# marvinli00/genie2

Measured on AMD Instinct MI355X. Metric: denoise-steps/sec (N=256, T=1000, batch=8), higher is better.
Workload: dtype f32 (pair-stack products as 3 f16 MFMAs on 2xf16-split operands, f32 accumulate); 1 GPU; unconditional N=256, T=1000, batch=8 per GPU, random-init base Denoiser (15.7M params), scale=0.6, reverse-loop steps 995..676; parallelism=replica per GPU x1, no data-path collective

## Files before the change

### genie2_amd/csrc/genie_api.hip

```cpp
#include <stdio.h>
#include <stdlib.h>
#include <string.h>
#include <math.h>
#include <algorithm>
#include <cmath>
#include <new>
#include <string>
#include <vector>

#include "common.h"

void pair_kernels_init();
void pair_fused_kernels_init();
void single_kernels_init(const genie_dims_t& d, int n_max);
void launch_scale_copy(genie_ctx* h, hipStream_t st, const float* in, float* out, int n, float s);
size_t ipa_attn_lds(const genie_dims_t& d, int N);

static char g_create_err[512] = "";

void set_handle_free_error(const char* msg) { snprintf(g_create_err, sizeof g_create_err, "%s", msg); }

#define SET_ERR(h, ...) do { snprintf((h)->err, sizeof((h)->err), __VA_ARGS__); } while (0)
#define HIP_TRY(h, call) do { hipError_t e_ = (call); if (e_ != hipSuccess) { \
    SET_ERR(h, "%s failed: %s (%s:%d)", #call, hipGetErrorString(e_), __FILE__, __LINE__); return GENIE_E_HIP; } } while (0)
// ... 100 lines not shown
static void free_batch(genie_ctx* h) {
    if (h->ws) { (void)hipFree(h->ws); h->ws = nullptr; h->ws_bytes = 0; }
    h->have_feats = false;
}

void genie_destroy(genie_handle_t h) {
    if (!h) return;
    (void)hipSetDevice(h->device);
    free_batch(h);
    train_ws_free(h);
    if (h->wdev) (void)hipFree(h->wdev);
    if (h->hxdev) (void)hipFree(h->hxdev);
    if (h->pos_tab) (void)hipFree(h->pos_tab);
    free(h->sched_host);
    for (int i = 0; i < h->prof_n; ++i) { (void)hipEventDestroy(h->prof_recs[i].a); (void)hipEventDestroy(h->prof_recs[i].b); }
    free(h->prof_recs);
    if (h->st2) { (void)hipStreamSynchronize(h->st2); (void)hipEventDestroy(h->ev_fork); (void)hipEventDestroy(h->ev_join); (void)hipStreamDestroy(h->st2); }
    delete[] h->pair;
    delete[] h->st;
    delete h;
}

const char* genie_last_error(genie_handle_t h) { return h ? h->err : g_create_err; }
size_t genie_workspace_bytes(genie_handle_t h) { return h ? h->ws_bytes : 0; }

namespace {
struct Img {
    std::vector<float> data;
    size_t add(size_t n) {
        const size_t off = (data.size() + 63) & ~(size_t)63;
        data.resize(off + n, 0.f);
        return off;
    }
    size_t raw(const float* src, size_t n) { const size_t o = add(n); memcpy(&data[o], src, n * sizeof(float)); return o; }
    size_t pack(const float* W, int rows, int cols) {
        const int NB = (rows + 31) / 32, KB = (cols + 7) / 8;
        const size_t o = add((size_t)NB * KB * 256);
        float* p = &data[o];
        for (int nb = 0; nb < NB; ++nb)
            for (int kb = 0; kb < KB; ++kb)
                for (int lane = 0; lane < 64; ++lane)
                    for (int e = 0; e < 4; ++e) {
                        const int r = nb * 32 + (lane & 31), k = kb * 8 + 4 * (lane >> 5) + e;
                        p[(((size_t)nb * KB + kb) * 64 + lane) * 4 + e] = (r < rows && k < cols) ? W[(size_t)r * cols + k] : 0.f;
                    }
        return o;
    }
};
uint16_t f2h(float f) {
    uint32_t x; memcpy(&x, &f, 4);
    const uint16_t sign = (uint16_t)((x >> 16) & 0x8000);
    x &= 0x7FFFFFFFu;
    if (x >= 0x7F800000u) return (uint16_t)(sign | (x > 0x7F800000u ? 0x7E00 : 0x7C00));
    if (x >= 0x477FF000u) return (uint16_t)(sign | 0x7C00);
    if (x < 0x38800000u) {
        float a; memcpy(&a, &x, 4);
        return (uint16_t)(sign | (uint16_t)nearbyintf(a * 16777216.0f));
    }
    const uint32_t mant = x & 0x7FFFFFu, rem = mant & 0x1FFFu;
    uint32_t r = (((x >> 23) - 112u) << 10) | (mant >> 13);
    if (rem > 0x1000u || (rem == 0x1000u && (r & 1u))) ++r;
    return (uint16_t)(sign | r);
}
float h2f(uint16_t v) {
    const int e = (v >> 10) & 31, m = v & 1023;
    float r = e == 0 ? ldexpf((float)m, -24) : e == 31 ? (m ? NAN : INFINITY) : ldexpf((float)(1024 + m), e - 25);
    return (v & 0x8000) ? -r : r;
}
float p2floor(double x) { return (x > 0 && std::isfinite(x)) ? (float)ldexp(1.0, (int)floor(log2(x))) : 1.0f; }
struct HxImg {
    std::vector<uint16_t> d;
    size_t begin() { d.resize((d.size() + 127) & ~(size_t)127); return d.size() * 2; }
    template <class F> void unit(F get) {
        const size_t o = d.size();
        d.resize(o + 1024);
        for (int lane = 0; lane < 64; ++lane)
            for (int e = 0; e < 8; ++e) {
                const float v = get(lane & 31, lane >> 5, e);
                const uint16_t hi = f2h(v);
                d[o + lane * 8 + e] = hi;
                d[o + 512 + lane * 8 + e] = f2h(v - h2f(hi));
            }
    }
};
double max_abs(const float* w, size_t n) { double m = 0; for (size_t i = 0; i < n; ++i) m = std::max(m, (double)fabsf(w[i])); return m; }
double hx_bound(const float* W, const float* b, int rows, int cols) {
    double m = 0;
    for (int r = 0; r < rows; ++r) {
        double ss = 0;
        for (int k = 0; k < cols; ++k) ss += (double)W[(size_t)r * cols + k] * W[(size_t)r * cols + k];
        m = std::max(m, sqrt(ss * cols) + fabs((double)b[r]));
    }
    return m;
}
constexpr float HX_SX = 1024.0f;

struct Cur {
    const float* p; size_t left;
    const float* take(size_t n) { if (n > left) { left = 0; return nullptr; } const float* r = p; p += n; left -= n; return r; }
};
void fold_ln(std::vector<float>& W, std::vector<float>& b, int rows, int cols, const float* g, const float* beta) {
    for (int r = 0; r < rows; ++r) {
        double acc = b[r];
        for (int k = 0; k < cols; ++k) acc += (double)W[(size_t)r * cols + k] * beta[k];
        b[r] = (float)acc;
        for (int k = 0; k < cols; ++k) W[(size_t)r * cols + k] *= g[k];
    }
}
std::vector<float> vcat(std::initializer_list<std::pair<const float*, size_t>> parts) {
    std::vector<float> v;
    for (auto& pr : parts) v.insert(v.end(), pr.first, pr.first + pr.second);
    return v;
}
}

int genie_load_weights(genie_handle_t h, const float* blob, size_t n_floats) {
    if (!h || !blob) return GENIE_E_ARG;
    const genie_dims_t& d = h->d;
    if (n_floats != genie_weight_count(&d)) {
        SET_ERR(h, "genie_load_weights: got %zu floats, dims need %zu", n_floats, genie_weight_count(&d));
        return GENIE_E_ARG;
    }
    HIP_TRY(h, hipSetDevice(h->device));
    const size_t cs = d.c_s, cp = d.c_p, ch = d.c_hidden_mul;
    Cur c{blob, n_floats};
    Img img;
    HxImg hx;
    std::vector<std::pair<float**, size_t>> fix;
    std::vector<std::pair<const unsigned char**, size_t>> hxfix;
    auto slot = [&](float** s, size_t off) { fix.push_back({s, off}); };
    struct GemmFix { float** slot; size_t hx_off; float inv_s; };
    std::vector<GemmFix> gfix;
    auto pack_gemm = [&](float** s, const float* W, int rows, int cols) {
        slot(s, img.pack(W, rows, cols));
        const float sw = p2floor(16384.0 / max_abs(W, (size_t)rows * cols));
        gfix.push_back({s, hx.begin(), 1.0f / sw});
        const int NB = (rows + 31) / 32, KC = (cols + 15) / 16;
        for (int nb = 0; nb < NB; ++nb)
            for (int kc = 0; kc < KC; ++kc)
                hx.unit([&](int j, int hh, int e) {
                    const int r = 32 * nb + j, k = 16 * kc + 8 * hh + e;
                    return (r < rows && k < cols) ? W[(size_t)r * cols + k] * sw : 0.f; });
    };

    size_t ones_off, zeros_off;
    {
        std::vector<float> one(512, 1.f), zero(512, 0.f);
        ones_off = img.raw(one.data(), one.size());
        zeros_off = img.raw(zero.data(), zero.size());
    }
    const int nsi = single_in(d);
    pack_gemm(&h->single_w, c.take(cs * nsi), (int)cs, nsi);
    {
        const float* wi = c.take(cp * cs);
        const float* wj = c.take(cp * cs);
        auto v = vcat({{wi, cp * cs}, {wj, cp * cs}});
        pack_gemm(&h->pij_w, v.data(), (int)(2 * cp), (int)cs);
    }
    {
        const int nr = 2 * d.relpos_k + 3;
        const float* w = c.take(cp * nr);
        std::vector<float> t((size_t)nr * cp);
        for (int o = 0; o < (int)cp; ++o) for (int k = 0; k < nr; ++k) t[(size_t)k * cp + o] = w[(size_t)o * nr + k];
        slot(&h->relpos_t, img.raw(t.data(), t.size()));
    }
    {
// ... 62 lines not shown
                        for (int kc = 0; kc < 8; ++kc) {
                            const std::vector<float>& m = (st & 1) ? zw : gw;
                            const float sc = (st & 1) ? szo : sgo;
                            const size_t ob = 2 * (st >> 1) + obl;
                            hx.unit([&](int j, int hh, int e) { return m[(32 * ob + j) * cp + 16 * kc + 8 * hh + e] * sc; });
                        }
                std::vector<float> bp(4 * ch), bgs(cp), bzs(cp);
                for (size_t r = 0; r < 4 * ch; ++r) bp[r] = bb[r] * HX_SX * (r < 2 * ch ? sp : sg);
                for (size_t r = 0; r < cp; ++r) { bgs[r] = gb[r] * HX_SX * sgo; bzs[r] = zb[r] * HX_SX * szo; }
                slot(&X.bias_proj, img.raw(bp.data(), bp.size()));
                slot(&X.bgs, img.raw(bgs.data(), cp)); slot(&X.bzs, img.raw(bzs.data(), cp));
                tm_save[2 * l + dir] = TmSave{w, gw, zw, sp, sg, sgo, szo};
            }
            slot(&T.ln_in_g, ones_off); slot(&T.ln_in_b, zeros_off);
            slot(&T.ln_out_g, ones_off); slot(&T.ln_out_b, zeros_off);
        }
        for (int node = 0; node < (d.n_head_tri > 0 ? 2 : 0); ++node) {
            TriAttW& A = node == 0 ? L.ta_start : L.ta_end;
            const size_t hc = (size_t)d.n_head_tri * d.c_hidden_tri_att;
            const float* ln_g = c.take(cp); const float* ln_b = c.take(cp);
            const float* b_w = c.take(d.n_head_tri * cp);
            const float* q_w = c.take(hc * cp); const float* k_w = c.take(hc * cp); const float* v_w = c.take(hc * cp);
            const float* o_w = c.take(cp * hc); const float* o_b = c.take(cp);
            const float* g_w = c.take(hc * cp); const float* g_b = c.take(hc);
            if (!g_b) { SET_ERR(h, "genie_load_weights: blob too short"); return GENIE_E_ARG; }
            slot(&A.ln_g, img.raw(ln_g, cp)); slot(&A.ln_b, img.raw(ln_b, cp));
            slot(&A.wb, img.raw(b_w, d.n_head_tri * cp));
            auto w = vcat({{q_w, hc * cp}, {k_w, hc * cp}, {v_w, hc * cp}, {g_w, hc * cp}});
            std::vector<float> bv(4 * hc, 0.f);
            memcpy(&bv[3 * hc], g_b, hc * sizeof(float));
            pack_gemm(&A.proj_w, w.data(), (int)(4 * hc), (int)cp);
            slot(&A.proj_b, img.raw(bv.data(), bv.size()));
            pack_gemm(&A.out_w, o_w, (int)cp, (int)hc); slot(&A.out_b, img.raw(o_b, cp));
            auto scale_of = [&](const float* W) {
                std::vector<float> wf(W, W + hc * cp), bf(hc, 0.f);
                fold_ln(wf, bf, (int)hc, (int)cp, ln_g, ln_b);
                return p2floor(32768.0 / hx_bound(wf.data(), bf.data(), (int)hc, (int)cp));
            };
            A.sq = scale_of(q_w); A.sk = scale_of(k_w); A.sv = scale_of(v_w);
        }
        const size_t nh = (size_t)d.pair_transition_n * cp;
        const float* lg = c.take(cp); const float* lb = c.take(cp);
        const float* w1 = c.take(nh * cp); const float* b1 = c.take(nh);
        const float* w2 = c.take(cp * nh); const float* b2 = c.take(cp);
        {
            std::vector<float> w1v(w1, w1 + nh * cp), b1v(b1, b1 + nh);
            fold_ln(w1v, b1v, (int)nh, (int)cp, lg, lb);
            slot(&L.pt_ln_g, ones_off); slot(&L.pt_ln_b, zeros_off);
            slot(&L.pt_w1, img.pack(w1v.data(), (int)nh, (int)cp)); slot(&L.pt_b1, img.raw(b1v.data(), nh));
            HxTransW& X = L.hx_pt;
            const float s1 = p2floor(16384.0 / max_abs(w1v.data(), nh * cp)), s2 = p2floor(16384.0 / max_abs(w2, cp * nh));
            const float sh = p2floor(32768.0 / hx_bound(w1v.data(), b1v.data(), (int)nh, (int)cp));
            X.sx = HX_SX; X.c1 = sh / (HX_SX * s1); X.c2 = 1.0f / (sh * s2);
            hxfix.push_back({&X.img, hx.begin()});
            for (size_t hb = 0; hb < nh / 32; ++hb) {
                for (int kc = 0; kc < 8; ++kc)
                    hx.unit([&](int i, int hh, int e) { return w1v[(32 * hb + i) * cp + 16 * kc + 8 * hh + e] * s1; });
                for (int cc = 0; cc < 2; ++cc)
                    for (int ob = 0; ob < 4; ++ob)
                        hx.unit([&](int j, int hh, int e) {
                            return w2[(size_t)(32 * ob + j) * nh + 32 * hb + 16 * cc + (e & 3) + 8 * (e >> 2) + 4 * hh] * s2; });
            }
            std::vector<float> b1s(nh), b2s(cp);
            for (size_t r = 0; r < nh; ++r) b1s[r] = b1v[r] * HX_SX * s1;
            for (size_t r = 0; r < cp; ++r) b2s[r] = b2[r] * sh * s2;
            slot(&X.b1s, img.raw(b1s.data(), nh)); slot(&X.b2s, img.raw(b2s.data(), cp));
            pt_save[l] = PtSave{w1v, std::vector<float>(w2, w2 + cp * nh), s1, s2};
        }
        slot(&L.pt_w2, img.pack(w2, (int)cp, (int)nh)); slot(&L.pt_b2, img.raw(b2, cp));
    }
    {
        auto ck = [](int kc, int hh, int e) { return 16 * kc + (e & 3) + 8 * (e >> 2) + 4 * hh; };
        auto emit_O = [&](const TmSave& t) {
            for (int which = 0; which < 2; ++which)
                for (int st = 0; st < 2; ++st)
                    for (int obl = 0; obl < 2; ++obl)
                        for (int kc = 0; kc < 8; ++kc) {
                            const std::vector<float>& m = which == 0 ? t.zw : t.gw;
                            const float sc = which == 0 ? t.szo : t.sgo;
                            const size_t ob = 2 * st + obl;
                            hx.unit([&](int i, int hh, int e) { return m[(32 * ob + i) * cp + ck(kc, hh, e)] * sc; });
                        }
        };
        auto emit_T = [&](const PtSave& t) {
            const size_t nh = (size_t)d.pair_transition_n * cp;
            for (size_t hb = 0; hb < nh / 32; ++hb) {
                for (int kc = 0; kc < 8; ++kc)
                    hx.unit([&](int i, int hh, int e) { return t.w1v[(32 * hb + i) * cp + ck(kc, hh, e)] * t.s1; });
                for (int cc = 0; cc < 2; ++cc)
                    for (int ob = 0; ob < 4; ++ob)
                        hx.unit([&](int j, int hh, int e) { return t.w2[(size_t)(32 * ob + j) * nh + 32 * hb + ck(cc, hh, e)] * t.s2; });
            }
        };
        auto emit_P = [&](const TmSave& t) {
            for (size_t pass = 0; pass < 8; ++pass)
                for (int kc = 0; kc < 8; ++kc) {
                    hx.unit([&](int i, int hh, int e) { return t.w[(32 * pass + i) * cp + ck(kc, hh, e)] * t.sp; });
                    hx.unit([&](int i, int hh, int e) { return t.w[(2 * ch + 32 * pass + i) * cp + ck(kc, hh, e)] * t.sg; });
                }
        };
        for (int l = 0; l < d.n_pair_transform_layer; ++l) {
            hxfix.push_back({&h->pair[l].fa.img, hx.begin()});
            emit_O(tm_save[2 * l]); emit_P(tm_save[2 * l + 1]);
            hxfix.push_back({&h->pair[l].fb.img, hx.begin()});
            emit_O(tm_save[2 * l + 1]); emit_T(pt_save[l]);
            if (l + 1 < d.n_pair_transform_layer) emit_P(tm_save[2 * l + 2]);
        }
    }
    const size_t H = d.n_head_ipa, C = d.c_hidden_ipa, Pq = d.n_qk_point, Pv = d.n_v_point;
    const size_t ncat = ipa_cat_n(d);
    std::vector<float> wb_all, bb_all;
    for (int l = 0; l < d.n_structure_layer; ++l) {
        StructLayerW& S = h->st[l];
        const float* hw = c.take(H);
        const float* q_w = c.take(H * C * cs);            const float* q_b = c.take(H * C);
        const float* kv_w = c.take(2 * H * C * cs);       const float* kv_b = c.take(2 * H * C);
        const float* qp_w = c.take(3 * H * Pq * cs);      const float* qp_b = c.take(3 * H * Pq);
        const float* kp_w = c.take(3 * H * (Pq + Pv) * cs); const float* kp_b = c.take(3 * H * (Pq + Pv));
        const float* b_w = c.take(H * cp);                const float* b_b = c.take(H);
        const float* o_w = c.take(cs * ncat);             const float* o_b = c.take(cs);
        const float* li_g = c.take(cs); const float* li_b = c.take(cs);
        const float* t1w = c.take(cs * cs); const float* t1b = c.take(cs);
        const float* t2w = c.take(cs * cs); const float* t2b = c.take(cs);
        const float* t3w = c.take(cs * cs); const float* t3b = c.take(cs);
        const float* lt_g = c.take(cs); const float* lt_b = c.take(cs);
        const float* bw = c.take(6 * cs); const float* bbs = c.take(6);
        if (!bbs) { SET_ERR(h, "genie_load_weights: blob too short"); return GENIE_E_ARG; }
        slot(&S.head_w, img.raw(hw, H));
        auto w = vcat({{q_w, H * C * cs}, {kv_w, 2 * H * C * cs}, {qp_w, 3 * H * Pq * cs}, {kp_w, 3 * H * (Pq + Pv) * cs}});
        auto bv = vcat({{q_b, H * C}, {kv_b, 2 * H * C}, {qp_b, 3 * H * Pq}, {kp_b, 3 * H * (Pq + Pv)}});
        pack_gemm(&S.proj_w, w.data(), ipa_proj_n(d), (int)cs);
        slot(&S.proj_b, img.raw(bv.data(), bv.size()));
        wb_all.insert(wb_all.end(), b_w, b_w + H * cp);
        bb_all.insert(bb_all.end(), b_b, b_b + H);
        pack_gemm(&S.out_w, o_w, (int)cs, (int)ncat); slot(&S.out_b, img.raw(o_b, cs));
        slot(&S.ln_ipa_g, img.raw(li_g, cs)); slot(&S.ln_ipa_b, img.raw(li_b, cs));
        pack_gemm(&S.t1_w, t1w, (int)cs, (int)cs); slot(&S.t1_b, img.raw(t1b, cs));
        pack_gemm(&S.t2_w, t2w, (int)cs, (int)cs); slot(&S.t2_b, img.raw(t2b, cs));
        pack_gemm(&S.t3_w, t3w, (int)cs, (int)cs); slot(&S.t3_b, img.raw(t3b, cs));
        slot(&S.ln_tr_g, img.raw(lt_g, cs)); slot(&S.ln_tr_b, img.raw(lt_b, cs));
        slot(&S.bb_w, img.raw(bw, 6 * cs)); slot(&S.bb_b, img.raw(bbs, 6));
    }
    pack_gemm(&h->ipa_bias_w, wb_all.data(), (int)(d.n_structure_layer * H), (int)cp);
    slot(&h->ipa_bias_b, img.raw(bb_all.data(), bb_all.size()));
    if (c.left != 0) { SET_ERR(h, "genie_load_weights: %zu floats left over", c.left); return GENIE_E_ARG; }

    if (h->wdev) { (void)hipFree(h->wdev); h->wdev = nullptr; }
    img.add(64);
    HIP_TRY(h, hipMalloc((void**)&h->wdev, img.data.size() * sizeof(float)));
    HIP_TRY(h, hipMemcpy(h->wdev, img.data.data(), img.data.size() * sizeof(float), hipMemcpyHostToDevice));
    h->wdev_floats = img.data.size();
    for (auto& f : fix) *f.first = h->wdev + f.second;
    if (h->hxdev) { (void)hipFree(h->hxdev); h->hxdev = nullptr; }
    hx.begin();
    HIP_TRY(h, hipMalloc((void**)&h->hxdev, hx.d.size() * 2 + 256));
    HIP_TRY(h, hipMemcpy(h->hxdev, hx.d.data(), hx.d.size() * 2, hipMemcpyHostToDevice));
    for (auto& f : hxfix) *f.first = h->hxdev + f.second;
    h->n_hxg = 0;
    const int hxg_cap = (int)(sizeof(h->hxg) / sizeof(h->hxg[0]));
    if ((int)gfix.size() > hxg_cap) { SET_ERR(h, "genie_load_weights: %zu row-GEMM weights exceed the %d hx image slots", gfix.size(), hxg_cap); return GENIE_E_ARG; }
    for (auto& g : gfix) h->hxg[h->n_hxg++] = HxGemmW{*g.slot, h->hxdev + g.hx_off, g.inv_s};
    h->have_weights = true;
    return GENIE_OK;
}

int genie_set_tables(genie_handle_t h, const float* pos_tab, int n_pos, const float* chain_tab, int n_chain,
                     const float* t_tab, const float* sched) {
    if (!h || !pos_tab || !chain_tab || !t_tab || !sched || n_pos < 1 || n_chain < 1) return GENIE_E_ARG;
    HIP_TRY(h, hipSetDevice(h->device));
    const genie_dims_t& d = h->d;
    const size_t T1 = d.n_timestep + 1;
    const size_t a = (size_t)n_pos * d.c_pos_emb, b = (size_t)n_chain * d.c_chain_emb, c = T1 * d.c_timestep_emb, s = 4 * T1;
    if (h->pos_tab) (void)hipFree(h->pos_tab);
    HIP_TRY(h, hipMalloc((void**)&h->pos_tab, (a + b + c + s) * sizeof(float)));
// ... 374 lines not shown
```

### genie2_amd/csrc/hx.h

```cpp
#pragma once
#include "common.h"

#ifdef __HIPCC__
typedef _Float16 h8 __attribute__((ext_vector_type(8)));
typedef _Float16 h2 __attribute__((ext_vector_type(2)));
typedef unsigned u32x4 __attribute__((ext_vector_type(4)));

#define MFH(a, b, c) c = __builtin_amdgcn_mfma_f32_32x32x16_f16(a, b, c, 0, 0, 0)
#define MFH3(ah, al, bh, bl, c) do { MFH(al, bh, c); MFH(ah, bl, c); MFH(ah, bh, c); } while (0)

__device__ __forceinline__ void hx_split2(float a, float b, float s, unsigned& hi, unsigned& lo) {
    asm("v_fma_mixlo_f16 %0, %1, %2, 0" : "=v"(hi) : "v"(a), "v"(s));
    asm("v_fma_mixhi_f16 %0, %1, %2, 0" : "+v"(hi) : "v"(b), "v"(s));
    asm("v_fma_mixlo_f16 %0, %1, %2, -%3 op_sel_hi:[0,0,1]" : "=v"(lo) : "v"(a), "v"(s), "v"(hi));
    asm("v_fma_mixhi_f16 %0, %1, %2, -%3 op_sel:[0,0,1] op_sel_hi:[0,0,1]" : "+v"(lo) : "v"(b), "v"(s), "v"(hi));
}
__device__ __forceinline__ void hx_split8(const float (&x)[8], float s, h8& hi, h8& lo) {
    u32x4 h, l;
    unsigned a, b;
    hx_split2(x[0], x[1], s, a, b); h.x = a; l.x = b;
    hx_split2(x[2], x[3], s, a, b); h.y = a; l.y = b;
    hx_split2(x[4], x[5], s, a, b); h.z = a; l.z = b;
    hx_split2(x[6], x[7], s, a, b); h.w = a; l.w = b;
    hi = __builtin_bit_cast(h8, h);
    lo = __builtin_bit_cast(h8, l);
}
__device__ __forceinline__ unsigned hx_pack_prod(float u, float t) {
    unsigned w;
    asm("v_fma_mixlo_f16 %0, %1, %2, 0" : "=v"(w) : "v"(u), "v"(t));
    asm("v_fma_mixhi_f16 %0, %1, %2, -%0 op_sel_hi:[0,0,1]" : "+v"(w) : "v"(u), "v"(t));
    return w;
}
__device__ __forceinline__ h8 hx_frag(const unsigned char* stage, int u, int part, int lane) {
    return *reinterpret_cast<const h8*>(stage + u * 2048 + part * 1024 + lane * 16);
}
#endif

#define HX_STAGE_BYTES 32768
#define HX_UNITS 16
```

### genie2_amd/csrc/hx_fused.h

```cpp
#pragma once
#include "hx_pair.h"

#define FZ_SB_BZ 0
#define FZ_SB_BG 128
#define FZ_SB_B1 256
#define FZ_SB_B2 768
#define FZ_SB_BP 896
#define FZ_SB_FLOATS 1408
#define FZ_OOR 0x7FFFFFF0
#define FZ_COMPILER_FENCE() asm volatile("" ::: "memory")

struct FusedArgs {
    float* z; const float* xcm; const float* rmask; const unsigned char* wimg;
    const float *bzs, *bgs, *b1s, *b2s, *bproj;
    unsigned *acm, *bcm;
    int N, NP, n_wtiles, n_hb;
    unsigned cm_bytes, z_bytes;
    float sx, cgo, cz, c1, c2, inv_c2, cpa, cpb, cg;
    int rev;
};

__device__ __forceinline__ void fz_zt_read(float4 (&raw)[16], const unsigned char* zt, int pl, int h, int half) {
#pragma unroll
    for (int q = 0; q < 4; ++q) {
        const int g = 4 * q + h;
        raw[2 * (4 * half + q)] = *reinterpret_cast<const float4*>(zt + pl * 256 + ((g ^ (pl & 15)) << 4));
        raw[2 * (4 * half + q) + 1] = *reinterpret_cast<const float4*>(zt + pl * 256 + (((g + 2) ^ (pl & 15)) << 4));
    }
}

__device__ __forceinline__ void fz_zt_chunk(float4& a, float4& b, const unsigned char* zt, int pl, int h, int q) {
    const int g = 4 * q + h;
    a = *reinterpret_cast<const float4*>(zt + pl * 256 + ((g ^ (pl & 15)) << 4));
    b = *reinterpret_cast<const float4*>(zt + pl * 256 + (((g + 2) ^ (pl & 15)) << 4));
}

__device__ __forceinline__ void fz_store_half(rsrc_t rz, unsigned char* zt, const f32x16& v0, const f32x16& v1, int lane, int soff,
                                              int row_stride, int nvalid, int hf) {
    const int pl = lane & 31, h = lane >> 5;
    FZ_COMPILER_FENCE();
#pragma unroll
    for (int q = 0; q < 4; ++q) {
        const f32x16& v = (q < 2) ? v0 : v1;
        const int r0 = 8 * (q & 1);
        const int g = 4 * q + h;
        *reinterpret_cast<float4*>(zt + pl * 256 + ((g ^ (pl & 15)) << 4)) = make_float4(v[r0], v[r0 + 1], v[r0 + 2], v[r0 + 3]);
        *reinterpret_cast<float4*>(zt + pl * 256 + (((g + 2) ^ (pl & 15)) << 4)) = make_float4(v[r0 + 4], v[r0 + 5], v[r0 + 6], v[r0 + 7]);
    }
    hx_lds_done();
#pragma unroll
    for (int j = 0; j < 8; ++j) {
        const int r = 4 * j + (lane >> 4);
        u32x4 d = *reinterpret_cast<const u32x4*>(zt + j * 1024 + lane * 16);
        const int g = (lane & 15) ^ (r & 15);
        const int voff = r < nvalid ? r * row_stride + (g << 4) : FZ_OOR;
        __builtin_amdgcn_raw_buffer_store_b128(d, rz, voff, soff + hf * 256, 0);
        asm volatile("s_nop 1" : "+v"(d) : : "memory");
    }
    FZ_COMPILER_FENCE();
}

__device__ __forceinline__ void fz_stats(const f32x16 (&v)[4], float sx, float& mean, float& sc) {
    float s = 0.f;
#pragma unroll
    for (int ob = 0; ob < 4; ++ob)
#pragma unroll
        for (int r = 0; r < 16; ++r) s += v[ob][r];
    s += __shfl_xor(s, 32);
    mean = s * (1.0f / 128.0f);
    float ss = 0.f;
#pragma unroll
    for (int ob = 0; ob < 4; ++ob)
#pragma unroll
        for (int r = 0; r < 16; ++r) { const float d = v[ob][r] - mean; ss += d * d; }
    ss += __shfl_xor(ss, 32);
    sc = sx / sqrtf(ss * (1.0f / 128.0f) + GENIE_LN_EPS);
}
__device__ __forceinline__ void fz_split_tile(h8 (&zh)[8], h8 (&zl)[8], const f32x16 (&v)[4], float mean, float sc) {
#pragma unroll
    for (int c = 0; c < 8; ++c) {
        float x[8];
#pragma unroll
        for (int e = 0; e < 8; ++e) x[e] = v[c >> 1][8 * (c & 1) + e] - mean;
        hx_split8(x, sc, zh[c], zl[c]);
    }
}
```

### genie2_amd/csrc/pair_fused_kernels.hip

```cpp
#include <string.h>
#include "hx_fused.h"

#define FZ_LDS_BYTES (2 * HX_STAGE_BYTES + 6144 + 8 * HX_ZT_BYTES)

template <bool COL, bool HAS_T, bool HAS_P = true>
__global__ __launch_bounds__(512, 1) void k_pair_fused(const FusedArgs A) {
    extern __shared__ __attribute__((aligned(16))) unsigned char smb[];
    float* sb = reinterpret_cast<float*>(smb + 2 * HX_STAGE_BYTES);
    const int lane = threadIdx.x & 63, wave = UNI(threadIdx.x >> 6);
    const int h = lane >> 5, pl = lane & 31;
    const int N = A.N, NP = A.NP, n_wtiles = A.n_wtiles;
    const int ntile = (N + 31) >> 5;
    const int n_tiles = (n_wtiles + 7) / 8;
    const int rev = A.rev;
    const int n_hb = HAS_T ? A.n_hb : 0;
    const int PBASE = 4 + n_hb;
    const rsrc_t rw = hx_rsrc(A.wimg, (unsigned)((PBASE + (HAS_P ? 8 : 0)) * HX_STAGE_BYTES));
    const rsrc_t rx = hx_rsrc(A.xcm, A.cm_bytes), rz = hx_rsrc(A.z, A.z_bytes);
    const rsrc_t ra = hx_rsrc(A.acm, A.cm_bytes), rb = hx_rsrc(A.bcm, A.cm_bytes);
    const int lane16 = lane * 16;
    const int sstride = NP * NP * 4;
    const int zstride = COL ? N * 512 : 512;
    auto issue = [&](int s, int buf) {
        if (wave >= 4) {
// ... 96 lines not shown
#pragma unroll
                        for (int q = 0; q < 4; ++q) fz_zt_chunk(rz1[2 * q], rz1[2 * q + 1], zt, pl_t, h_t, q);
                    }
                    if (half == 0 && kc == 2) { hx_lds_done(); hx_zt_dma(rz, zt, lane_t, zsoff, zstride, znv, 0); }
                    if (half == 1 && kc == 1) {
                        zsh = __shfl(rz1[0].x, lane & 31);
#pragma unroll
                        for (int q = 0; q < 8; ++q) {
                            const float a = rz1[q].x - zsh, bq = rz1[q].y - zsh, c = rz1[q].z - zsh, d = rz1[q].w - zsh;
                            zs1 += (a + bq) + (c + d); zs2 += (a * a + bq * bq) + (c * c + d * d);
                        }
                    }
                    if (half == 1 && kc >= 2 && kc <= 5) {
                        float4 ta, tb;
                        fz_zt_chunk(ta, tb, zt, pl_t, h_t, kc - 2);
                        const float a = ta.x - zsh, bq = ta.y - zsh, c = ta.z - zsh, d = ta.w - zsh;
                        const float e = tb.x - zsh, f = tb.y - zsh, g = tb.z - zsh, hh = tb.w - zsh;
                        zs1 += ((a + bq) + (c + d)) + ((e + f) + (g + hh));
                        zs2 += ((a * a + bq * bq) + (c * c + d * d)) + ((e * e + f * f) + (g * g + hh * hh));
                    }
                }
                hx_stage_landed();
                hx_stage_barrier();
            }
            zs1 += __shfl_xor(zs1, 32); zs2 += __shfl_xor(zs2, 32);
            const float zm_s = zs1 * (1.0f / 128.0f);
            const float zmean = zsh + zm_s;
            const float zsc = A.sx / sqrtf(fmaxf(zs2 * (1.0f / 128.0f) - zm_s * zm_s, 0.f) + GENIE_LN_EPS);
#pragma unroll
            for (int half = 0; half < 2; ++half) {
                if (half == 0) issue(3, 1);
                else issue(4, 0);
                const unsigned char* stage = smb + half * HX_STAGE_BYTES;
                f32x16 ga, gb;
#pragma unroll
                for (int r = 0; r < 16; ++r) {
                    ga[r] = sbt[FZ_SB_BG + (2 * half) * 32 + acc_row(r, lane)];
                    gb[r] = sbt[FZ_SB_BG + (2 * half + 1) * 32 + acc_row(r, lane)];
                }
                h8 f0 = hx_frag(stage, 0, 0, lane), f0l = hx_frag(stage, 0, 1, lane), f1 = hx_frag(stage, 8, 0, lane),
                   f1l = hx_frag(stage, 8, 1, lane);
#pragma unroll
                for (int kc = 0; kc < 8; ++kc) {
                    const int kn = min(kc + 1, 7);
                    const h8 n0 = hx_frag(stage, kn, 0, lane), n0l = hx_frag(stage, kn, 1, lane), n1 = hx_frag(stage, 8 + kn, 0, lane),
                             n1l = hx_frag(stage, 8 + kn, 1, lane);
                    float4 ca, cb;
                    if (kc < 4) fz_zt_chunk(ca, cb, zt, pl_t, h_t, kc);
                    else { ca = rz1[2 * (kc - 4)]; cb = rz1[2 * (kc - 4) + 1]; }
                    const float xz[8] = {ca.x - zmean, ca.y - zmean, ca.z - zmean, ca.w - zmean, cb.x - zmean, cb.y - zmean, cb.z - zmean, cb.w - zmean};
                    h8 sh, sl;
                    hx_split8(xz, zsc, sh, sl);
                    PIPE_FENCE();
                    MFH3(f0, f0l, sh, sl, ga);
                    MFH3(f1, f1l, sh, sl, gb);
                    PIPE_FENCE();
                    f0 = n0; f0l = n0l; f1 = n1; f1l = n1l;
                }
                float4 res[8];
                if (half == 0) {
#pragma unroll
                    for (int q = 0; q < 4; ++q) fz_zt_chunk(res[2 * q], res[2 * q + 1], zt, pl_t, h_t, q);
                } else {
#pragma unroll
                    for (int q = 0; q < 8; ++q) res[q] = rz1[q];
                }
#pragma unroll
                for (int r = 0; r < 16; ++r) {
                    const float g0 = A.cz * __builtin_amdgcn_rcpf(1.0f + __builtin_amdgcn_exp2f(ga[r] * A.cgo));
                    const float g1 = A.cz * __builtin_amdgcn_rcpf(1.0f + __builtin_amdgcn_exp2f(gb[r] * A.cgo));
                    const float4 za = res[2 * (r >> 3) + ((r & 7) >> 2)], zb = res[2 * (2 + (r >> 3)) + ((r & 7) >> 2)];
                    const float z0 = (r & 3) == 0 ? za.x : (r & 3) == 1 ? za.y : (r & 3) == 2 ? za.z : za.w;
                    const float z1 = (r & 3) == 0 ? zb.x : (r & 3) == 1 ? zb.y : (r & 3) == 2 ? zb.z : zb.w;
                    v[2 * half][r] = fmaf(v[2 * half][r], g0, z0);
                    v[2 * half + 1][r] = fmaf(v[2 * half + 1][r], g1, z1);
                }
                hx_stage_landed();
                hx_stage_barrier();
            }
        }

        h8 zh[8], zl[8];
        if constexpr (HAS_T) {
            float mean, sc;
            fz_stats(v, A.sx, mean, sc);
            fz_split_tile(zh, zl, v, mean, sc);
#pragma unroll
            for (int ob = 0; ob < 4; ++ob)
#pragma unroll
                for (int r = 0; r < 16; ++r) v[ob][r] = fmaf(v[ob][r], A.inv_c2, sbt[FZ_SB_B2 + ob * 32 + acc_row(r, lane)]);
            f32x16 d;
#pragma unroll
            for (int r = 0; r < 16; ++r) d[r] = sbt[FZ_SB_B1 + acc_row(r, lane)];
            auto t_stage = [&](int hb) {
                if (HAS_P || hb + 1 < n_hb) issue(4 + hb + 1, (hb + 1) & 1);
                else if (more) issue(0, 0);
                const unsigned char* stage = smb + (hb & 1) * HX_STAGE_BYTES;
                {
                    h8 wh = hx_frag(stage, 0, 0, lane), wl = hx_frag(stage, 0, 1, lane);
#pragma unroll
                    for (int kc = 0; kc < 8; ++kc) {
                        const h8 nh = hx_frag(stage, min(kc + 1, 7), 0, lane), nl = hx_frag(stage, min(kc + 1, 7), 1, lane);
                        PIPE_FENCE();
                        MFH3(wh, wl, zh[kc], zl[kc], d);
                        PIPE_FENCE();
                        wh = nh; wl = nl;
                    }
                }
                h8 ah[2], al[2];
#pragma unroll
                for (int c = 0; c < 2; ++c) {
                    float x[8];
#pragma unroll
                    for (int e = 0; e < 8; ++e) x[e] = fmaxf(d[8 * c + e], 0.f);
                    hx_split8(x, A.c1, ah[c], al[c]);
                }
                {
                    h8 bh = hx_frag(stage, 8, 0, lane), bl = hx_frag(stage, 8, 1, lane);
#pragma unroll
                    for (int u = 0; u < 8; ++u) {
                        const h8 nh = hx_frag(stage, 8 + min(u + 1, 7), 0, lane), nl = hx_frag(stage, 8 + min(u + 1, 7), 1, lane);
                        PIPE_FENCE();
                        MFH3(bh, bl, ah[u >> 2], al[u >> 2], v[u & 3]);
                        PIPE_FENCE();
                        bh = nh; bl = nl;
                        if (u == 1) {
#pragma unroll
                            for (int r = 0; r < 16; ++r) d[r] = sbt[FZ_SB_B1 + (hb + 1) * 32 + acc_row(r, lane)];
                        }
                    }
                }
                hx_stage_landed();
                hx_stage_barrier();
            };
#pragma unroll 1
            for (int hb = 0; hb < n_hb; ++hb) t_stage(hb);
            const float m2 = msk * A.c2;
#pragma unroll
            for (int ob = 0; ob < 4; ++ob)
#pragma unroll
                for (int r = 0; r < 16; ++r) v[ob][r] *= m2;
        }

        fz_store_half(rz, zt, v[0], v[1], lane_t, zsoff, zstride, nvalid, 0);
        FZ_COMPILER_FENCE();
        fz_store_half(rz, zt, v[2], v[3], lane_t, zsoff, zstride, nvalid, 1);
        FZ_COMPILER_FENCE();
        if constexpr (HAS_P) {
            float mean, sc;
            fz_stats(v, A.sx, mean, sc);
            fz_split_tile(zh, zl, v, mean, sc);
        }
        hx_lds_done();
        if constexpr (!HAS_P) {
            if (more) hx_zt_dma(rz, zt, lane_t, n_zsoff, zstride, n_nv, 1);
        }

        if constexpr (HAS_P) {
            const float* sbias = sbt + FZ_SB_BP;
            const float cg = A.cg;
            const float ma = msk * A.cpa, mb = msk * A.cpb;
            const int voff = (pl < nvalid) ? (4 * h * NP * NP + pl) * 4 : FZ_OOR;
            const int sbase = ((b * 128 * NP + line) * NP + t0i) * 4;
            unsigned wst[8];
            f32x16 apA, agA, apB, agB;
#pragma unroll
            for (int r = 0; r < 16; ++r) { apB[r] = 0.f; agB[r] = 0.f; apA[r] = sbias[acc_row(r, lane)]; agA[r] = sbias[256 + acc_row(r, lane)]; }
#pragma unroll 1
            for (int pp = 0; pp < 4; ++pp) {
                {
                    const int pass = 2 * pp;
                    issue(PBASE + pass + 1, 1);
                    const unsigned char* stage = smb;
                    const rsrc_t e_rd = pp > 2 ? rb : ra;
                    const int e_voff = pp == 0 ? FZ_OOR : voff;
                    const int e_so = sbase + ((pass - 1) & 3) * 32 * sstride;
                    const float e_pm = pp > 2 ? mb : ma;
                    HX_PROJ_STAGE(apA, agA, apB, agB);
                    asm volatile("s_waitcnt vmcnt(16)" ::: "memory");
                    if (more) {
                        if (pp == 2) hx_zt_dma(rz, zt, lane_t, n_zsoff, zstride, n_nv, 1, 0, 4);
                    }
                    hx_stage_barrier();
                }
                {
                    const int pass = 2 * pp + 1;
                    if (pp < 3) issue(PBASE + pass + 1, 0);
                    else if (more) issue(0, 0);
                    const unsigned char* stage = smb + HX_STAGE_BYTES;
                    const rsrc_t e_rd = pp < 2 ? ra : rb;
                    const int e_voff = voff;
                    const int e_so = sbase + ((pass - 1) & 3) * 32 * sstride;
                    const float e_pm = pp < 2 ? ma : mb;
                    HX_PROJ_STAGE(apB, agB, apA, agA);
                    asm volatile("s_waitcnt vmcnt(16)" ::: "memory");
                    if (more) {
                        if (pp == 2) hx_zt_dma(rz, zt, lane_t, n_zsoff, zstride, n_nv, 1, 4, 4);
                    }
                    hx_stage_barrier();
                }
            }
            {
                const rsrc_t e_rd = rb;
                const int e_voff = voff, e_so = sbase + 3 * 32 * sstride;
                const float e_pm = mb;
                float t[16], u[16];
#pragma unroll
                for (int r = 0; r < 16; ++r) {
                    HX_PROJ_PIECE_A(agB, r, t[r]);
                    HX_PROJ_PIECE_B(apB, r, t[r], u[r]);
                }
                PIPE_FENCE();
#pragma unroll
                for (int r = 0; r < 16; ++r) HX_PROJ_PIECE_C_NOW(r, t[r], u[r]);
            }
        }
    }
#undef FZ_XLOAD
}

static int fz_num_cu() {
    static int n = 0;
    if (!n) { int dev = 0; hipDeviceProp_t pr; (void)hipGetDevice(&dev); (void)hipGetDeviceProperties(&pr, dev); n = pr.multiProcessorCount > 0 ? pr.multiProcessorCount : 256; }
    return n;
}

void pair_fused_kernels_init() {
    (void)hipFuncSetAttribute(reinterpret_cast<const void*>(k_pair_fused<true, false>), hipFuncAttributeMaxDynamicSharedMemorySize, FZ_LDS_BYTES);
    (void)hipFuncSetAttribute(reinterpret_cast<const void*>(k_pair_fused<false, true>), hipFuncAttributeMaxDynamicSharedMemorySize, FZ_LDS_BYTES);
    (void)hipFuncSetAttribute(reinterpret_cast<const void*>(k_pair_fused<false, true, false>), hipFuncAttributeMaxDynamicSharedMemorySize, FZ_LDS_BYTES);
// ... 23 lines not shown
```

Measured before the change: 110.7 batch-steps/s.

## Switch pair transition MLP to 16x16x32 MFMAs with transposed tile layout

Rewrites the pair-transition stage of the fused pair kernel to use 16x16x32 f16 MFMAs instead of 32x32x16. The accumulator tile is transposed through LDS into a new per-lane layout, and the host-side weight packing is re-emitted in matching 16-row units. The result is written back from that layout, with a round trip through LDS to restore the old register layout when the following projection needs it. This adds LDS shuffles, lane shuffles for the per-row stats, and recomputes the mask per element; the aim is presumably a better MFMA rate or better latency hiding for this shape.

Result: no change. 111.5 batch-steps/s (median of 6 runs) (+0.7%).

```diff
diff --git a/genie2_amd/csrc/genie_api.hip b/genie2_amd/csrc/genie_api.hip
--- a/genie2_amd/csrc/genie_api.hip
+++ b/genie2_amd/csrc/genie_api.hip
@@ -206,6 +206,7 @@
                 d[o + 512 + lane * 8 + e] = f2h(v - h2f(hi));
             }
     }
+    template <class F> void unit16(F get) { unit([&](int i, int hh, int e) { return get(i & 15, 2 * hh + (i >> 4), e); }); }
 };
 double max_abs(const float* w, size_t n) { double m = 0; for (size_t i = 0; i < n; ++i) m = std::max(m, (double)fabsf(w[i])); return m; }
 double hx_bound(const float* W, const float* b, int rows, int cols) {
@@ -434,14 +435,15 @@
                             hx.unit([&](int i, int hh, int e) { return m[(32 * ob + i) * cp + ck(kc, hh, e)] * sc; });
                         }
         };
+        auto ck16 = [](int c, int g, int e) { return 32 * c + 16 * (e >> 2) + 4 * g + (e & 3); };
         auto emit_T = [&](const PtSave& t) {
             const size_t nh = (size_t)d.pair_transition_n * cp;
             for (size_t hb = 0; hb < nh / 32; ++hb) {
-                for (int kc = 0; kc < 8; ++kc)
-                    hx.unit([&](int i, int hh, int e) { return t.w1v[(32 * hb + i) * cp + ck(kc, hh, e)] * t.s1; });
-                for (int cc = 0; cc < 2; ++cc)
-                    for (int ob = 0; ob < 4; ++ob)
-                        hx.unit([&](int j, int hh, int e) { return t.w2[(size_t)(32 * ob + j) * nh + 32 * hb + ck(cc, hh, e)] * t.s2; });
+                for (int kc = 0; kc < 4; ++kc)
+                    for (int fb = 0; fb < 2; ++fb)
+                        hx.unit16([&](int i, int g, int e) { return t.w1v[(32 * hb + 16 * fb + i) * cp + ck16(kc, g, e)] * t.s1; });
+                for (int ob = 0; ob < 8; ++ob)
+                    hx.unit16([&](int j, int g, int e) { return t.w2[(size_t)(16 * ob + j) * nh + 32 * hb + ck16(0, g, e)] * t.s2; });
             }
         };
         auto emit_P = [&](const TmSave& t) {
diff --git a/genie2_amd/csrc/hx.h b/genie2_amd/csrc/hx.h
--- a/genie2_amd/csrc/hx.h
+++ b/genie2_amd/csrc/hx.h
@@ -8,6 +8,8 @@
 
 #define MFH(a, b, c) c = __builtin_amdgcn_mfma_f32_32x32x16_f16(a, b, c, 0, 0, 0)
 #define MFH3(ah, al, bh, bl, c) do { MFH(al, bh, c); MFH(ah, bl, c); MFH(ah, bh, c); } while (0)
+#define MFQ(a, b, c) c = __builtin_amdgcn_mfma_f32_16x16x32_f16(a, b, c, 0, 0, 0)
+#define MFQ3(ah, al, bh, bl, c) do { MFQ(al, bh, c); MFQ(ah, bl, c); MFQ(ah, bh, c); } while (0)
 
 __device__ __forceinline__ void hx_split2(float a, float b, float s, unsigned& hi, unsigned& lo) {
     asm("v_fma_mixlo_f16 %0, %1, %2, 0" : "=v"(hi) : "v"(a), "v"(s));
diff --git a/genie2_amd/csrc/hx_fused.h b/genie2_amd/csrc/hx_fused.h
--- a/genie2_amd/csrc/hx_fused.h
+++ b/genie2_amd/csrc/hx_fused.h
@@ -35,6 +35,8 @@
     b = *reinterpret_cast<const float4*>(zt + pl * 256 + (((g + 2) ^ (pl & 15)) << 4));
 }
 
+__device__ __forceinline__ void fz_store_pieces(rsrc_t rz, unsigned char* zt, int lane, int soff, int row_stride, int nvalid, int hf);
+
 __device__ __forceinline__ void fz_store_half(rsrc_t rz, unsigned char* zt, const f32x16& v0, const f32x16& v1, int lane, int soff,
                                               int row_stride, int nvalid, int hf) {
     const int pl = lane & 31, h = lane >> 5;
@@ -47,6 +49,77 @@
         *reinterpret_cast<float4*>(zt + pl * 256 + ((g ^ (pl & 15)) << 4)) = make_float4(v[r0], v[r0 + 1], v[r0 + 2], v[r0 + 3]);
         *reinterpret_cast<float4*>(zt + pl * 256 + (((g + 2) ^ (pl & 15)) << 4)) = make_float4(v[r0 + 4], v[r0 + 5], v[r0 + 6], v[r0 + 7]);
     }
+    fz_store_pieces(rz, zt, lane, soff, row_stride, nvalid, hf);
+}
+
+
+__device__ __forceinline__ int acc_row_b(int i, int lane) { return 4 * (lane >> 4) + i; }
+
+__device__ __forceinline__ void fz_to_b(f32x4 (&w)[8][2], unsigned char* zt, const f32x16& v0, const f32x16& v1, int lane, int hf) {
+    const int pl = lane & 31, h = lane >> 5, n = lane & 15, gb = lane >> 4;
+    FZ_COMPILER_FENCE();
+#pragma unroll
+    for (int q = 0; q < 4; ++q) {
+        const f32x16& v = (q < 2) ? v0 : v1;
+        const int r0 = 8 * (q & 1);
+        const int g = 4 * q + h;
+        *reinterpret_cast<float4*>(zt + pl * 256 + ((g ^ (pl & 15)) << 4)) = make_float4(v[r0], v[r0 + 1], v[r0 + 2], v[r0 + 3]);
+        *reinterpret_cast<float4*>(zt + pl * 256 + (((g + 2) ^ (pl & 15)) << 4)) = make_float4(v[r0 + 4], v[r0 + 5], v[r0 + 6], v[r0 + 7]);
+    }
+    hx_lds_done();
+#pragma unroll
+    for (int fbl = 0; fbl < 4; ++fbl)
+#pragma unroll
+        for (int q = 0; q < 2; ++q) {
+            const int row = 2 * n + q;
+            w[4 * hf + fbl][q] = *reinterpret_cast<const f32x4*>(zt + row * 256 + (((4 * fbl + gb) ^ (row & 15)) << 4));
+        }
+    hx_lds_done();
+    FZ_COMPILER_FENCE();
+}
+
+template <bool BACK>
+__device__ __forceinline__ void fz_store_half_b(rsrc_t rz, unsigned char* zt, const f32x4 (&w)[8][2], f32x16& v0, f32x16& v1, int lane, int soff,
+                                                int row_stride, int nvalid, int hf) {
+    const int pl = lane & 31, h = lane >> 5, n = lane & 15, gb = lane >> 4;
+    FZ_COMPILER_FENCE();
+#pragma unroll
+    for (int fbl = 0; fbl < 4; ++fbl)
+#pragma unroll
+        for (int q = 0; q < 2; ++q) {
+            const int row = 2 * n + q;
+            *reinterpret_cast<f32x4*>(zt + row * 256 + (((4 * fbl + gb) ^ (row & 15)) << 4)) = w[4 * hf + fbl][q];
+        }
+    fz_store_pieces(rz, zt, lane, soff, row_stride, nvalid, hf);
+    if (BACK) {
+#pragma unroll
+        for (int q = 0; q < 4; ++q) {
+            f32x16& v = (q < 2) ? v0 : v1;
+            const int r0 = 8 * (q & 1);
+            const int g = 4 * q + h;
+            const float4 a = *reinterpret_cast<const float4*>(zt + pl * 256 + ((g ^ (pl & 15)) << 4));
+            const float4 b = *reinterpret_cast<const float4*>(zt + pl * 256 + (((g + 2) ^ (pl & 15)) << 4));
+            v[r0] = a.x; v[r0 + 1] = a.y; v[r0 + 2] = a.z; v[r0 + 3] = a.w;
+            v[r0 + 4] = b.x; v[r0 + 5] = b.y; v[r0 + 6] = b.z; v[r0 + 7] = b.w;
+        }
+        hx_lds_done();
+        FZ_COMPILER_FENCE();
+    }
+}
+
+__device__ __forceinline__ void fz_split_tile_b(h8 (&zh)[4][2], h8 (&zl)[4][2], const f32x4 (&w)[8][2], const float (&mean)[2], const float (&sc)[2]) {
+#pragma unroll
+    for (int c = 0; c < 4; ++c)
+#pragma unroll
+        for (int q = 0; q < 2; ++q) {
+            float x[8];
+#pragma unroll
+            for (int e = 0; e < 8; ++e) x[e] = w[2 * c + (e >> 2)][q][e & 3] - mean[q];
+            hx_split8(x, sc[q], zh[c][q], zl[c][q]);
+        }
+}
+
+__device__ __forceinline__ void fz_store_pieces(rsrc_t rz, unsigned char* zt, int lane, int soff, int row_stride, int nvalid, int hf) {
     hx_lds_done();
 #pragma unroll
     for (int j = 0; j < 8; ++j) {
diff --git a/genie2_amd/csrc/pair_fused_kernels.hip b/genie2_amd/csrc/pair_fused_kernels.hip
--- a/genie2_amd/csrc/pair_fused_kernels.hip
+++ b/genie2_amd/csrc/pair_fused_kernels.hip
@@ -202,16 +202,30 @@
 
         h8 zh[8], zl[8];
         if constexpr (HAS_T) {
-            float mean, sc;
-            fz_stats(v, A.sx, mean, sc);
-            fz_split_tile(zh, zl, v, mean, sc);
-#pragma unroll
-            for (int ob = 0; ob < 4; ++ob)
-#pragma unroll
-                for (int r = 0; r < 16; ++r) v[ob][r] = fmaf(v[ob][r], A.inv_c2, sbt[FZ_SB_B2 + ob * 32 + acc_row(r, lane)]);
-            f32x16 d;
-#pragma unroll
-            for (int r = 0; r < 16; ++r) d[r] = sbt[FZ_SB_B1 + acc_row(r, lane)];
+            f32x4 w[8][2];
+            float mean[2], sc[2];
+            {
+                float m1, s1;
+                fz_stats(v, A.sx, m1, s1);
+                mean[0] = __shfl(m1, 2 * (lane & 15)); mean[1] = __shfl(m1, 2 * (lane & 15) + 1);
+                sc[0] = __shfl(s1, 2 * (lane & 15)); sc[1] = __shfl(s1, 2 * (lane & 15) + 1);
+            }
+            fz_to_b(w, zt, v[0], v[1], lane_t, 0);
+            fz_to_b(w, zt, v[2], v[3], lane_t, 1);
+            h8 bzh[4][2], bzl[4][2];
+            fz_split_tile_b(bzh, bzl, w, mean, sc);
+#pragma unroll
+            for (int fb = 0; fb < 8; ++fb)
+#pragma unroll
+                for (int i = 0; i < 4; ++i) {
+                    const float b2 = sbt[FZ_SB_B2 + fb * 16 + acc_row_b(i, lane)];
+                    w[fb][0][i] = fmaf(w[fb][0][i], A.inv_c2, b2); w[fb][1][i] = fmaf(w[fb][1][i], A.inv_c2, b2);
+                }
+            f32x4 d[2][2];
+#pragma unroll
+            for (int fb = 0; fb < 2; ++fb)
+#pragma unroll
+                for (int i = 0; i < 4; ++i) d[fb][0][i] = d[fb][1][i] = sbt[FZ_SB_B1 + fb * 16 + acc_row_b(i, lane)];
             auto t_stage = [&](int hb) {
                 if (HAS_P || hb + 1 < n_hb) issue(4 + hb + 1, (hb + 1) & 1);
                 else if (more) issue(0, 0);
@@ -219,21 +233,22 @@
                 {
                     h8 wh = hx_frag(stage, 0, 0, lane), wl = hx_frag(stage, 0, 1, lane);
 #pragma unroll
-                    for (int kc = 0; kc < 8; ++kc) {
-                        const h8 nh = hx_frag(stage, min(kc + 1, 7), 0, lane), nl = hx_frag(stage, min(kc + 1, 7), 1, lane);
+                    for (int u = 0; u < 8; ++u) {
+                        const h8 nh = hx_frag(stage, min(u + 1, 7), 0, lane), nl = hx_frag(stage, min(u + 1, 7), 1, lane);
                         PIPE_FENCE();
-                        MFH3(wh, wl, zh[kc], zl[kc], d);
+                        MFQ3(wh, wl, bzh[u >> 1][0], bzl[u >> 1][0], d[u & 1][0]);
+                        MFQ3(wh, wl, bzh[u >> 1][1], bzl[u >> 1][1], d[u & 1][1]);
                         PIPE_FENCE();
                         wh = nh; wl = nl;
                     }
                 }
                 h8 ah[2], al[2];
 #pragma unroll
-                for (int c = 0; c < 2; ++c) {
+                for (int q = 0; q < 2; ++q) {
                     float x[8];
 #pragma unroll
-                    for (int e = 0; e < 8; ++e) x[e] = fmaxf(d[8 * c + e], 0.f);
-                    hx_split8(x, A.c1, ah[c], al[c]);
+                    for (int e = 0; e < 8; ++e) x[e] = fmaxf(d[e >> 2][q][e & 3], 0.f);
+                    hx_split8(x, A.c1, ah[q], al[q]);
                 }
                 {
                     h8 bh = hx_frag(stage, 8, 0, lane), bl = hx_frag(stage, 8, 1, lane);
@@ -241,12 +256,15 @@
                     for (int u = 0; u < 8; ++u) {
                         const h8 nh = hx_frag(stage, 8 + min(u + 1, 7), 0, lane), nl = hx_frag(stage, 8 + min(u + 1, 7), 1, lane);
                         PIPE_FENCE();
-                        MFH3(bh, bl, ah[u >> 2], al[u >> 2], v[u & 3]);
+                        MFQ3(bh, bl, ah[0], al[0], w[u][0]);
+                        MFQ3(bh, bl, ah[1], al[1], w[u][1]);
                         PIPE_FENCE();
                         bh = nh; bl = nl;
                         if (u == 1) {
 #pragma unroll
-                            for (int r = 0; r < 16; ++r) d[r] = sbt[FZ_SB_B1 + (hb + 1) * 32 + acc_row(r, lane)];
+                            for (int fb = 0; fb < 2; ++fb)
+#pragma unroll
+                                for (int i = 0; i < 4; ++i) d[fb][0][i] = d[fb][1][i] = sbt[FZ_SB_B1 + (hb + 1) * 32 + fb * 16 + acc_row_b(i, lane)];
                         }
                     }
                 }
@@ -255,17 +273,25 @@
             };
 #pragma unroll 1
             for (int hb = 0; hb < n_hb; ++hb) t_stage(hb);
-            const float m2 = msk * A.c2;
-#pragma unroll
-            for (int ob = 0; ob < 4; ++ob)
-#pragma unroll
-                for (int r = 0; r < 16; ++r) v[ob][r] *= m2;
-        }
-
-        fz_store_half(rz, zt, v[0], v[1], lane_t, zsoff, zstride, nvalid, 0);
-        FZ_COMPILER_FENCE();
-        fz_store_half(rz, zt, v[2], v[3], lane_t, zsoff, zstride, nvalid, 1);
-        FZ_COMPILER_FENCE();
+#pragma unroll
+            for (int q = 0; q < 2; ++q) {
+                const int pb = 2 * (lane & 15) + q;
+                const float m2 = ((pb < nvalid) ? A.rmask[b * N + line] * A.rmask[b * N + t0i + pb] : 0.f) * A.c2;
+#pragma unroll
+                for (int fb = 0; fb < 8; ++fb)
+#pragma unroll
+                    for (int i = 0; i < 4; ++i) w[fb][q][i] *= m2;
+            }
+            fz_store_half_b<HAS_P>(rz, zt, w, v[0], v[1], lane_t, zsoff, zstride, nvalid, 0);
+            FZ_COMPILER_FENCE();
+            fz_store_half_b<HAS_P>(rz, zt, w, v[2], v[3], lane_t, zsoff, zstride, nvalid, 1);
+            FZ_COMPILER_FENCE();
+        } else {
+            fz_store_half(rz, zt, v[0], v[1], lane_t, zsoff, zstride, nvalid, 0);
+            FZ_COMPILER_FENCE();
+            fz_store_half(rz, zt, v[2], v[3], lane_t, zsoff, zstride, nvalid, 1);
+            FZ_COMPILER_FENCE();
+        }
         if constexpr (HAS_P) {
             float mean, sc;
             fz_stats(v, A.sx, mean, sc);
```
